# HJakeCunningham/ASVGP

Hardware: AMD Instinct MI355X
Metric: Mpoints/s per ELBO+grad step, N=10M 1D Matern-3/2 M=2048 (higher is better)
Workload: dtype f64

## Files before the change

asvgp_amd/csrc/bcr_mfma.hpp:

```cpp
#pragma once
#include "bcr.hpp"
#include "prior_plan.hpp"

namespace asvgp {

constexpr int BM_THREADS = 1024;
constexpr int BM_B = 4;
constexpr int BM_GAT = 0, BM_GBT = 16, BM_DINV = 32, BM_SD = 48, BM_CAT = 64, BM_CBT = 80, BM_W = 96, BM_DG = 100, BM_REC = 104;

__host__ __device__ inline size_t bcr_mfma_ws_doubles(long nb) { return (size_t)nb * BM_REC + 64; }
__host__ __device__ inline size_t bcr_mfma_lds_doubles(long nb) {
  return (size_t)((nb + 1) / 2 + 1) * 32 + (size_t)nb * 4 + 96 + (size_t)(BM_THREADS / 64) * 4 * 40 + (size_t)(nb / 8 + 2) * 52;
}

__device__ __forceinline__ double bm_mfma(double a, double b, double c) { return __builtin_amdgcn_mfma_f64_4x4x4f64(a, b, c, 0, 0, 0); }

__device__ __forceinline__ double bm_chol_linv(const double (&d)[10], int hi, int lo, double& dprod, int& badj) {
  double l00, i0, l10, l20, l30, l11, i1, l21, l31, l22, i2, l32, l33, i3;
  Num<double>::sqrt_inv(d[0], l00, i0);
  badj = !(d[0] > 0.0) ? 1 : 0;
  l10 = d[1] * i0; l20 = d[3] * i0; l30 = d[6] * i0;
  double s = fma(-l10, l10, d[2]);
  badj = (!(s > 0.0) && !badj) ? 2 : badj;
  Num<double>::sqrt_inv(s, l11, i1);
  l21 = fma(-l20, l10, d[4]) * i1;
  l31 = fma(-l30, l10, d[7]) * i1;
  s = fma(-l21, l21, fma(-l20, l20, d[5]));
  badj = (!(s > 0.0) && !badj) ? 3 : badj;
  Num<double>::sqrt_inv(s, l22, i2);
  l32 = fma(-l31, l21, fma(-l30, l20, d[8])) * i2;
  s = fma(-l32, l32, fma(-l31, l31, fma(-l30, l30, d[9])));
  badj = (!(s > 0.0) && !badj) ? 4 : badj;
  Num<double>::sqrt_inv(s, l33, i3);
  dprod = (l00 * l11) * (l22 * l33);
  const double z0 = (lo == 0) ? i0 : 0.0;
  const double z1 = fma(-l10, z0, (lo == 1) ? 1.0 : 0.0) * i1;
  const double z2 = fma(-l21, z1, fma(-l20, z0, (lo == 2) ? 1.0 : 0.0)) * i2;
  const double z3 = fma(-l32, z2, fma(-l31, z1, fma(-l30, z0, (lo == 3) ? 1.0 : 0.0))) * i3;
  return hi == 0 ? z0 : (hi == 1 ? z1 : (hi == 2 ? z2 : z3));
}

template <typename Src> __device__ __forceinline__ auto bm_src_load(const Src& A, int dd, long col, long M, int) -> decltype(A.load_dc(dd, col, M)) {
  return A.load_dc(dd, col, M);
}
template <typename Src> __device__ __forceinline__ double bm_src_load(const Src& A, int dd, long col, long M, long) {
  return A.load((long)dd * M + col, true);
}
struct BmLog {
  double m; int e;
  __device__ __forceinline__ void mul(double p) {
    m *= p;
    const int hi = __double2hiint(m);
    e += ((hi >> 20) & 0x7ff) - 1023;
    m = __hiloint2double((hi & 0x800fffff) | 0x3ff00000, __double2loint(m));
  }
};

__device__ __forceinline__ unsigned long long bm_wave_xor(unsigned long long x) {
#pragma unroll
  for (int off = 32; off > 0; off >>= 1) x ^= (unsigned long long)__shfl_xor((long long)x, off, 64);
  return x;
}
__device__ __forceinline__ void bm_msg_send(double* box, int n, double v, unsigned long long tag, int lane) {
  unsigned long long* b = reinterpret_cast<unsigned long long*>(box);
  const unsigned long long w = lane < n ? (unsigned long long)__double_as_longlong(v) : 0ull;
  const unsigned long long x = bm_wave_xor(w) ^ tag;
  if (lane < n) __hip_atomic_store(b + lane, w, __ATOMIC_RELAXED, __HIP_MEMORY_SCOPE_AGENT);
  if (lane == n) __hip_atomic_store(b + n, x, __ATOMIC_RELAXED, __HIP_MEMORY_SCOPE_AGENT);
}
__device__ __forceinline__ bool bm_msg_recv(const double* box, int n, double& v, unsigned long long tag, int lane, long spin_limit) {
  const unsigned long long* b = reinterpret_cast<const unsigned long long*>(box);
  for (long spins = 0; spins <= spin_limit; ++spins) {
    const unsigned long long w = lane <= n ? __hip_atomic_load(b + lane, __ATOMIC_RELAXED, __HIP_MEMORY_SCOPE_AGENT) : 0ull;
    const unsigned long long x = bm_wave_xor(lane < n ? w : 0ull) ^ tag;
    const unsigned long long chk = (unsigned long long)__shfl((long long)w, n, 64);
    if (x == chk) { v = __longlong_as_double((long long)w); return true; }
    __builtin_amdgcn_s_sleep(1);
  }
  return false;
}

struct BmSplit {
  int half = -1;
  double* xchg = nullptr;
  long spin_limit = 0;
  int* gave_up = nullptr;
  unsigned long long tag = 0;
};
constexpr int BM_XCHG = 96;

template <typename Src>
__device__ __attribute__((always_inline)) void bcr_mfma_solve(Src A, const double* rhs, int M, double* ws, double* lds, double* Sband, double* x,
                                                              double* logdet, int* info, int rhs_stride = 1, double* stamps = nullptr,
                                                              BmSplit sp = BmSplit{}) {
  constexpr int B = BM_B;
  const int tid = threadIdx.x;
  const int lane = tid & 63, wv = __builtin_amdgcn_readfirstlane(tid >> 6);
  const int r = lane >> 4, q = (lane >> 2) & 3, c = lane & 3;
  const int e = r * 4 + c, et = c * 4 + r;
  const int hi = r > c ? r : c, lo = r > c ? c : r;
  const int nb = (M + B - 1) / B;
  const int nslot = (nb + 1) / 2;
  double* Dl = lds;
  double* El = lds + (size_t)(nslot + 1) * 16;
  double* xs = El + (size_t)(nslot + 1) * 16;
  double* red = xs + (size_t)nb * B;
  double* slab = red + 96 + (size_t)(wv * 4 + q) * 40;
  double* Fl = red + 96 + (size_t)(BM_THREADS / 64) * 4 * 40;
  double* Sl = lds;
  int levels = 0;
  while ((1 << levels) < nb) ++levels;
  const bool split = sp.half >= 0;
  const int top = levels - 1, ht = 1 << (top > 0 ? top : 0);
  double s_other = 0.0;
  int bad_other = 0x7fffffff;
  auto level_share = [&](int l, int ne, int& m0, int& ne_h) {
    m0 = 0; ne_h = ne;
    if (!split) return;
    if (l < top) {
      const int mL = ht >> (l + 1);
      if (sp.half == 0) ne_h = ne < mL ? ne : mL;
      else { m0 = mL; ne_h = ne > mL ? ne - mL : 0; }
    } else {
      ne_h = sp.half == 0 ? ne : 0;
    }
  };
  int bad = 0;
  BmLog ld{1.0, 0};
  unsigned long long t_prev = stamps ? __builtin_amdgcn_s_memtime() : 0ull;
  int nst = 0;
  auto stamp = [&]() {
    if (stamps && tid == 0) { const unsigned long long t = __builtin_amdgcn_s_memtime(); stamps[nst++] = (double)(t - t_prev); t_prev = t; }
  };
  auto rec = [&](int node) -> double* { return ws + (size_t)node * BM_REC; };
  auto bandD = [&](int n, int rr, int cc) -> double {
    const int col = n * B + cc, row = n * B + rr;
    const bool pad = row >= M;
    const double v = bm_src_load(A, rr - cc, pad ? 0 : col, (long)M, 0);
    return pad ? ((rr == cc) ? 1.0 : 0.0) : v;
  };
  auto bandE = [&](int n, int rr, int cc) -> double {
    if (rr > cc) return 0.0;
    const int col = n * B + cc, row = (n + 1) * B + rr;
    const bool pad = row >= M;
    const double v = bm_src_load(A, B + rr - cc, pad ? 0 : col, (long)M, 0);
    return pad ? 0.0 : v;
  };
  if ((nb & 1) && tid < 16 && !(split && sp.half == 0)) {
    const int rr = tid >> 2, cc = tid & 3;
    Dl[(size_t)((nb - 1) >> 1) * 16 + tid] = bandD(nb - 1, rr > cc ? rr : cc, rr > cc ? cc : rr);
  }
  if (split && sp.half == 0 && tid < 16) Dl[(size_t)(ht >> 1) * 16 + tid] = 0.0;
  for (int row = tid; row < nb * B; row += BM_THREADS) {
    const bool sep_left = split && sp.half == 0 && row >= ht * B && row < (ht + 1) * B;
    xs[row] = (row < M && !sep_left) ? rhs[(long)row * rhs_stride] : 0.0;
  }
  __syncthreads();
  stamp();

  constexpr int RMAXR = 4;
  for (int l = 0; l < levels; ++l) {
    const int h = 1 << l;
    const int ne = (nb > h) ? (nb - h + 2 * h - 1) / (2 * h) : 0;
    int m0, ne_h;
    level_share(l, ne, m0, ne_h);
    if (split && l == top) {
      if (sp.half == 1) {
        if (wv == 0) {
          const double v = lane < 16 ? Dl[(size_t)(ht >> 1) * 16 + lane] : (lane < 20 ? xs[ht * B + lane - 16] : 0.0);
          bm_msg_send(sp.xchg, 20, v, sp.tag | 1ull, lane);
        }
        const double mine = (r == 0 && c == 0) ? (log(ld.m) + (double)ld.e * 0.6931471805599453094) : 0.0;
        const double tot = wave_sum_dpp(mine);
        int bm = bad ? bad : 0x7fffffff;
#pragma unroll
        for (int off = 32; off > 0; off >>= 1) { const int o = __shfl_xor(bm, off, 64); bm = o < bm ? o : bm; }
        int* sbad = reinterpret_cast<int*>(red + 32);
        if (lane == 0) { red[wv] = tot; sbad[wv] = bm; }
        __syncthreads();
        if (wv == 0) {
          double sv = 0.0;
          int bmin = 0x7fffffff;
          for (int w2 = 0; w2 < BM_THREADS / 64; ++w2) { sv += red[w2]; bmin = sbad[w2] < bmin ? sbad[w2] : bmin; }
          bm_msg_send(sp.xchg + 24, 2, lane == 0 ? sv : (double)bmin, sp.tag | 2ull, lane);
        }
      } else {
        if (wv == 0) {
          double v = 0.0;
          if (!bm_msg_recv(sp.xchg, 20, v, sp.tag | 1ull, lane, sp.spin_limit)) { if (lane == 0) *sp.gave_up = 1; }
          else {
            if (lane < 16) Dl[(size_t)(ht >> 1) * 16 + lane] += v;
            else if (lane < 20) xs[ht * B + lane - 16] += v;
          }
        }
        __syncthreads();
        if (*sp.gave_up) return;
      }
      stamp();
    }
    double updb[RMAXR], ybu[RMAXR];
    int qv = q, ev = e;
    asm volatile("" : "+v"(qv), "+v"(ev));
    double sl[2][3];
    auto slab_loads = [&](int rd0) __attribute__((always_inline)) {
#pragma unroll
      for (int u = 0; u < 2; ++u) {
#pragma unroll
        for (int t3 = 0; t3 < 3; ++t3) {
          sl[u][t3] = 0.0;
          int m = (rd0 + u) * 64 + wv * 4 + qv;
          m = m0 + (m < ne_h ? m : ne_h - 1);
          const int kk = ev + 16 * t3, dd = kk >> 3, col = m * 2 * B + (kk & 7);
          const bool in = kk < 40 && col + dd < M;
          const double v = bm_src_load(A, in ? dd : 0, in ? col : 0, (long)M, 0);
          sl[u][t3] = in ? v : ((dd == 0) ? 1.0 : 0.0);
        }
      }
    };
#pragma unroll
    for (int rd = 0; rd < RMAXR; ++rd) {
      __builtin_amdgcn_sched_barrier(0);
      if (l == 0 && (rd & 1) == 0) slab_loads(rd);
      updb[rd] = 0.0; ybu[rd] = 0.0;
      if (rd * 64 + wv * 4 >= ne_h) continue;
      const int ml = rd * 64 + wv * 4 + q;
      const bool act = ml < ne_h;
      const int i = h + (m0 + (act ? ml : ne_h - 1)) * 2 * h, a = i - h, b = i + h;
      const bool hasb = b < nb;
      const int bsafe = hasb ? b : a;
      double d[10];
      double ea, eb, da;
      if (l == 0) {
#pragma unroll
        for (int t3 = 0; t3 < 3; ++t3) if (e + 16 * t3 < 40) slab[e + 16 * t3] = sl[rd & 1][t3];
        int kk = 0;
#pragma unroll
        for (int rr = 0; rr < 4; ++rr)
#pragma unroll
          for (int cc = 0; cc <= rr; ++cc) d[kk++] = slab[(rr - cc) * 8 + 4 + cc];
        ea = slab[(4 + lo - hi) * 8 + hi];
        ea = (r <= c) ? ea : 0.0;
        eb = slab[(4 + lo - hi) * 8 + 4 + hi];
        eb = (hasb && c <= r) ? eb : 0.0;
        da = slab[(hi - lo) * 8 + lo];
      } else {
        const double* Di = Dl + (size_t)(i >> 1) * 16;
        int kk = 0;
#pragma unroll
        for (int rr = 0; rr < 4; ++rr)
#pragma unroll
          for (int cc = 0; cc <= rr; ++cc) d[kk++] = Di[rr * 4 + cc];
        ea = El[(size_t)(a >> 1) * 16 + e];
        eb = El[(size_t)(i >> 1) * 16 + et];
        eb = hasb ? eb : 0.0;
        da = Dl[(size_t)(a >> 1) * 16 + e];
      }
      double yv = xs[i * B + r], ya = xs[a * B + r];
      yv = (c == 0) ? yv : 0.0;
      ya = (c == 0) ? ya : 0.0;
      (void)bsafe;
      double dprod;
      int badj;
      const double t = bm_chol_linv(d, hi, lo, dprod, badj);
      if (act && badj && !bad) bad = i * B + badj;
      const double linv = (r >= c) ? t : 0.0;
      const double linvT = (c >= r) ? t : 0.0;
      if (act) ld.mul(dprod);
      const double ua = bm_mfma(linvT, ea, 0.0);
      const double ub = bm_mfma(linvT, eb, 0.0);
      const double zz = bm_mfma(linvT, yv, 0.0);
      const double nua = -ua, nub = -ub;
      const double da_new = bm_mfma(nua, ua, da);
      const double e_new = bm_mfma(nub, ua, 0.0);
      const double ya_new = bm_mfma(nua, zz, ya);
      updb[rd] = bm_mfma(ub, ub, 0.0);
      ybu[rd] = bm_mfma(ub, zz, 0.0);
      updb[rd] = act ? updb[rd] : 0.0;
      ybu[rd] = act ? ybu[rd] : 0.0;
      const double gat = bm_mfma(ua, linv, 0.0);
      const double gbt = bm_mfma(ub, linv, 0.0);
      const double dinv = bm_mfma(linv, linv, 0.0);
      const double w = bm_mfma(linv, zz, 0.0);
      if (act) {
        if (l >= 3) {
          double* R = Fl + (size_t)(i >> 3) * 52;
          R[e] = gat; R[16 + e] = gbt; R[32 + e] = dinv;
          if (c == 0) R[48 + r] = w;
        } else {
          double* R = rec(i);
          R[BM_GAT + e] = gat; R[BM_GBT + e] = gbt; R[BM_DINV + e] = dinv;
          if (c == 0) R[BM_W + r] = w;
        }
        Dl[(size_t)(a >> 1) * 16 + e] = da_new;
        El[(size_t)(a >> 1) * 16 + e] = e_new;
        if (c == 0) xs[a * B + r] = ya_new;
      }
    }
    bcr_lds_barrier();
#pragma unroll
    for (int rd = 0; rd < RMAXR; ++rd) {
      if (rd * 64 + wv * 4 >= ne_h) continue;
      const int ml = rd * 64 + wv * 4 + q;
      const int i = h + (m0 + ml) * 2 * h, b = i + h;
      if (ml < ne_h && b < nb) {
        Dl[(size_t)(b >> 1) * 16 + e] -= updb[rd];
        if (c == 0) xs[b * B + r] -= ybu[rd];
      }
    }
    bcr_lds_barrier();
    stamp();
  }
  if (wv == 0 && !(split && sp.half == 1)) {
    const bool act = q == 0;
    double d[10];
    int kk = 0;
#pragma unroll
    for (int rr = 0; rr < 4; ++rr)
#pragma unroll
      for (int cc = 0; cc <= rr; ++cc) { const double v = Dl[rr * 4 + cc]; d[kk++] = act ? v : ((rr == cc) ? 1.0 : 0.0); }
    const double yv = (act && c == 0) ? xs[r] : 0.0;
    double dprod;
    int badj;
    const double t = bm_chol_linv(d, hi, lo, dprod, badj);
    if (act && badj && !bad) bad = badj;
    const double linv = (r >= c) ? t : 0.0, linvT = (c >= r) ? t : 0.0;
    if (act) ld.mul(dprod);
    const double s00 = bm_mfma(linv, linv, 0.0);
    const double zz = bm_mfma(linvT, yv, 0.0);
    const double x0 = bm_mfma(linv, zz, 0.0);
    if (act) {
      rec(0)[BM_SD + e] = s00;
      Sl[e] = s00;
      if (r >= c && r < M) Sband[(long)(r - c) * M + c] = s00;
      if (c == 0) xs[r] = x0;
    }
  }
  __syncthreads();
  stamp();
  unsigned long long lw = 0ull;
  for (int l = levels - 1; l >= 0; --l) {
    const int h = 1 << l;
    const int ne = (nb > h) ? (nb - h + 2 * h - 1) / (2 * h) : 0;
    int m0, ne_h;
    level_share(l, ne, m0, ne_h);
    if (split && sp.half == 0 && wv == BM_THREADS / 64 - 1) {
      if (l == top - 1 && lane <= 2)
        lw = __hip_atomic_load(reinterpret_cast<const unsigned long long*>(sp.xchg + 24) + lane, __ATOMIC_RELAXED, __HIP_MEMORY_SCOPE_AGENT);
      if (l == 2) {
        const unsigned long long x = bm_wave_xor(lane < 2 ? lw : 0ull) ^ (sp.tag | 2ull);
        const unsigned long long chk = (unsigned long long)__shfl((long long)lw, 2, 64);
        double v = __longlong_as_double((long long)lw);
        bool ok = x == chk;
        if (!ok) ok = bm_msg_recv(sp.xchg + 24, 2, v, sp.tag | 2ull, lane, sp.spin_limit);
        if (!ok) { if (lane == 0) *sp.gave_up = 1; }
        else if (lane < 2) red[48 + lane] = v;
      }
    }
#pragma unroll
    for (int rd = 0; rd < RMAXR; ++rd) {
      __builtin_amdgcn_sched_barrier(0);
      if (rd * 64 + wv * 4 >= ne_h) continue;
      const int ml = rd * 64 + wv * 4 + q;
      const bool act = ml < ne_h;
      const int i = h + (m0 + (act ? ml : ne_h - 1)) * 2 * h, a = i - h, b = i + h;
      const bool hasb = b < nb;
      const int bs = hasb ? b : a;
      const bool e_is_a = ((a / (2 * h)) & 1) != 0;
      double gat, gbt, dinv, w, saa, sbb, sba, sab;
      if (l >= 3) {
        const double* R = Fl + (size_t)(i >> 3) * 52;
        gat = R[e]; gbt = R[16 + e]; dinv = R[32 + e]; w = R[48 + r];
      } else {
        const double* R = rec(i);
        gat = R[BM_GAT + e]; gbt = R[BM_GBT + e]; dinv = R[BM_DINV + e]; w = R[BM_W + r];
      }
      if (l >= 1) {
        const double* Ra = Sl + (size_t)(a >> 2) * 48;
        const double* Rb = Sl + (size_t)(bs >> 2) * 48;
        saa = Ra[e];
        sbb = Rb[e];
        sba = e_is_a ? Ra[32 + e] : Rb[16 + et];
        sab = e_is_a ? Ra[32 + et] : Rb[16 + e];
      } else {
        const double* Ra = rec(a);
        const double* Rb = rec(bs);
        saa = Ra[BM_SD + e];
        sbb = Rb[BM_SD + e];
        sba = e_is_a ? Ra[BM_CBT + e] : Rb[BM_CAT + et];
        sab = e_is_a ? Ra[BM_CBT + et] : Rb[BM_CAT + e];
      }
      sbb = hasb ? sbb : 0.0; sba = hasb ? sba : 0.0; sab = hasb ? sab : 0.0;
      double xa = xs[a * B + r], xb = xs[bs * B + r];
      xa = (c == 0) ? xa : 0.0;
      xb = (hasb && c == 0) ? xb : 0.0;
      w = (c == 0) ? w : 0.0;
      double ncat = bm_mfma(saa, gat, 0.0);
      ncat = bm_mfma(sba, gbt, ncat);
      double ncbt = bm_mfma(sab, gat, 0.0);
      ncbt = bm_mfma(sbb, gbt, ncbt);
      double sii = bm_mfma(ncat, gat, dinv);
      sii = bm_mfma(ncbt, gbt, sii);
      double gx = bm_mfma(gat, xa, 0.0);
      gx = bm_mfma(gbt, xb, gx);
      if (act) {
        if (c == 0) xs[i * B + r] = w - gx;
        if (l >= 2) {
          double* Rw = Sl + (size_t)(i >> 2) * 48;
          Rw[e] = sii; Rw[16 + e] = -ncat; Rw[32 + e] = -ncbt;
        }
        if (l > 0) {
          double* Rw = rec(i);
          Rw[BM_SD + e] = sii; Rw[BM_CAT + e] = -ncat; Rw[BM_CBT + e] = -ncbt;
        }
        if (r >= c && i * B + r < M) Sband[(long)(r - c) * M + i * B + c] = sii;
        if (l == 0) {
          if (c <= r && i * B + c < M) Sband[(long)(B + c - r) * M + a * B + r] = -ncat;
          if (hasb && r <= c && b * B + r < M) Sband[(long)(B + r - c) * M + i * B + c] = -ncbt;
        }
      }
    }
    if (l == 1) __syncthreads(); else bcr_lds_barrier();
    if (split && l == top) {
      double* Rs = Sl + (size_t)(ht >> 2) * 48;
      if (sp.half == 0) {
        if (wv == 0) bm_msg_send(sp.xchg + 32, 52, lane < 48 ? Rs[lane < 48 ? lane : 0] : (lane < 52 ? xs[ht * B + lane - 48] : 0.0), sp.tag | 3ull, lane);
      } else {
        if (wv == 0) {
          double v = 0.0;
          if (!bm_msg_recv(sp.xchg + 32, 52, v, sp.tag | 3ull, lane, sp.spin_limit)) { if (lane == 0) *sp.gave_up = 1; }
          else if (lane < 48) {
            Rs[lane] = v;
            rec(ht)[BM_SD + lane] = v;
            if (lane < 16) {
              const int rr = lane >> 2, cc = lane & 3;
              if (rr >= cc && ht * B + rr < M) Sband[(long)(rr - cc) * M + ht * B + cc] = v;
            }
          } else if (lane < 52) {
            xs[ht * B + lane - 48] = v;
          }
        }
        __syncthreads();
        if (*sp.gave_up) return;
      }
    }
    stamp();
  }
  if (!(split && sp.half == 0))
    for (int col = M - B + tid; col < M; col += BM_THREADS)
      if (col >= 0)
#pragma unroll
        for (int dd = 1; dd <= B; ++dd)
          if (col + dd >= M) Sband[(long)dd * M + col] = 0.0;
  {
    const int row0 = (split && sp.half == 1) ? (ht + 1) * B : 0, row1 = (split && sp.half == 0) ? (ht + 1) * B : M;
    for (int row = row0 + tid; row < row1 && row < M; row += BM_THREADS) x[(long)row * rhs_stride] = xs[row];
  }
  if (!(split && sp.half == 1)) {
    const double mine = (r == 0 && c == 0) ? (log(ld.m) + (double)ld.e * 0.6931471805599453094) : 0.0;
    const double tot = wave_sum_dpp(mine);
    int bm = bad ? bad : 0x7fffffff;
#pragma unroll
    for (int off = 32; off > 0; off >>= 1) { const int o = __shfl_xor(bm, off, 64); bm = o < bm ? o : bm; }
    int* sbad = reinterpret_cast<int*>(red + 32);
    if (lane == 0) { red[wv] = tot; sbad[wv] = bm; }
    __syncthreads();
    if (split && tid == 0) { s_other = red[48]; bad_other = (int)red[49]; }
    if (tid == 0) {
      double s = 0.0;
      int bmin = 0x7fffffff;
      for (int w2 = 0; w2 < BM_THREADS / 64; ++w2) { s += red[w2]; bmin = sbad[w2] < bmin ? sbad[w2] : bmin; }
      s += s_other;
      bmin = bad_other < bmin ? bad_other : bmin;
      __hip_atomic_store(logdet + 0, 2.0 * s, __ATOMIC_RELAXED, __HIP_MEMORY_SCOPE_AGENT);
      __hip_atomic_store(logdet + 1, 0.0, __ATOMIC_RELAXED, __HIP_MEMORY_SCOPE_AGENT);
      __hip_atomic_store(info, (bmin == 0x7fffffff) ? 0 : bmin, __ATOMIC_RELAXED, __HIP_MEMORY_SCOPE_AGENT);
    }
  }
  stamp();
}


__host__ __device__ inline size_t bcr_mfma_pre_ws_doubles(long nb) { return (size_t)nb * 96 + 64; }
__host__ __device__ inline size_t bcr_mfma_pre_lds_doubles(long nb, int n_rec) {
  return PRIOR_TAB_HEADER + (size_t)2 * n_rec * prior_rec_fields(BM_B) + (size_t)(nb / 4 + 2) * 96 + (size_t)(nb + 1) / 2 + 64;
}

struct BmDual { double v, d; };
__device__ __forceinline__ BmDual bm_dmfma(BmDual x, BmDual y, BmDual c) {
  BmDual r;
  r.v = bm_mfma(x.v, y.v, c.v);
  r.d = bm_mfma(x.d, y.v, c.d);
  r.d = bm_mfma(x.v, y.d, r.d);
  return r;
}

__device__ __attribute__((always_inline)) void bcr_mfma_backward_pre(const double* __restrict__ tab, int n_rec, const int* __restrict__ node_rec, int M,
                                                                      double* ws, double* lds, double* Sv, double* Sd, double* logdet, int* info,
                                                                      unsigned long long* done_flag, unsigned long long seq,
                                                                      const unsigned long long* ready_flag = nullptr, long spin_limit = 0, int* gave_up = nullptr) {
  constexpr int B = BM_B, W = prior_rec_fields(B);
  const int tid = threadIdx.x;
  if (ready_flag) {
    if (tid == 0) {
      long spins = 0;
      while (__hip_atomic_load(ready_flag, __ATOMIC_RELAXED, __HIP_MEMORY_SCOPE_SYSTEM) < seq) {
        __builtin_amdgcn_s_sleep(8);
        if (++spins > spin_limit) { *gave_up = 1; break; }
      }
    }
    __syncthreads();
    if (*gave_up) return;
    __builtin_amdgcn_fence(__ATOMIC_ACQUIRE, "");
  }
  const int lane = tid & 63, wv = __builtin_amdgcn_readfirstlane(tid >> 6);
  const int r = lane >> 4, q = (lane >> 2) & 3, c = lane & 3;
  const int e = r * 4 + c, et = c * 4 + r;
  const int nb = (M + B - 1) / B;
  const int n_tab = PRIOR_TAB_HEADER + 2 * n_rec * W;
  double* tl = lds;
  double* Sl = lds + n_tab;
  int* nrl = reinterpret_cast<int*>(Sl + (size_t)(nb / 4 + 2) * 96);
  {
    const double2* src = reinterpret_cast<const double2*>(tab);
    double2* dst = reinterpret_cast<double2*>(tl);
    for (int i2 = tid; i2 < n_tab / 2; i2 += BM_THREADS) dst[i2] = src[i2];
    for (int i2 = tid; i2 < nb; i2 += BM_THREADS) nrl[i2] = node_rec[i2];
  }
  __syncthreads();
  if (done_flag && tid == 0) __hip_atomic_store(done_flag, seq, __ATOMIC_RELAXED, __HIP_MEMORY_SCOPE_SYSTEM);
  const double* tv = tl + PRIOR_TAB_HEADER;
  const double* td = tv + (size_t)n_rec * W;
  int levels = 0;
  while ((1 << levels) < nb) ++levels;
  if (tid < 16) {
    const int r0 = nrl[0];
    const double xv = tv[(size_t)r0 * W + prior_f_UA(B) + tid], xd = td[(size_t)r0 * W + prior_f_UA(B) + tid];
    Sl[tid] = xv; Sl[48 + tid] = xd;
    ws[tid] = xv; ws[48 + tid] = xd;
    const int rr = tid >> 2, cc = tid & 3;
    if (rr >= cc && rr < M) { Sv[(long)(rr - cc) * M + cc] = xv; Sd[(long)(rr - cc) * M + cc] = xd; }
  }
  __syncthreads();
  constexpr int RMAXR = 4;
  for (int l = levels - 1; l >= 0; --l) {
    const int h = 1 << l;
    const int ne = (nb > h) ? (nb - h + 2 * h - 1) / (2 * h) : 0;
#pragma unroll
    for (int rd = 0; rd < RMAXR; ++rd) {
      __builtin_amdgcn_sched_barrier(0);
      if (rd * 64 + wv * 4 >= ne) continue;
      const int m = rd * 64 + wv * 4 + q;
      const bool act = m < ne;
      const int i = h + (act ? m : ne - 1) * 2 * h, a = i - h, b = i + h;
      const bool hasb = b < nb;
      const int bs = hasb ? b : a;
      const bool e_is_a = ((a / (2 * h)) & 1) != 0;
      const int ri = nrl[i];
      const double* fv = tv + (size_t)ri * W;
      const double* fd = td + (size_t)ri * W;
      const BmDual gat{fv[prior_f_GAT(B) + e], fd[prior_f_GAT(B) + e]};
      const BmDual gbt{fv[prior_f_GBT(B) + e], fd[prior_f_GBT(B) + e]};
      const BmDual dinv{fv[prior_f_DINV(B) + e], fd[prior_f_DINV(B) + e]};
      BmDual saa, sbb, sba, sab;
      if (l >= 1) {
        const double* Ra = Sl + (size_t)(a >> 2) * 96;
        const double* Rb = Sl + (size_t)(bs >> 2) * 96;
        saa = BmDual{Ra[e], Ra[48 + e]};
        sbb = BmDual{Rb[e], Rb[48 + e]};
        sba = e_is_a ? BmDual{Ra[32 + e], Ra[80 + e]} : BmDual{Rb[16 + et], Rb[64 + et]};
        sab = e_is_a ? BmDual{Ra[32 + et], Ra[80 + et]} : BmDual{Rb[16 + e], Rb[64 + e]};
      } else {
        const double* Ga = ws + (size_t)a * 96;
        const double* Gb = ws + (size_t)bs * 96;
        saa = BmDual{Ga[e], Ga[48 + e]};
        sbb = BmDual{Gb[e], Gb[48 + e]};
        sba = e_is_a ? BmDual{Ga[32 + e], Ga[80 + e]} : BmDual{Gb[16 + et], Gb[64 + et]};
        sab = e_is_a ? BmDual{Ga[32 + et], Ga[80 + et]} : BmDual{Gb[16 + e], Gb[64 + e]};
      }
      if (!hasb) { sbb = BmDual{0.0, 0.0}; sba = sbb; sab = sbb; }
      const BmDual zero{0.0, 0.0};
      BmDual ncat = bm_dmfma(saa, gat, zero);
      ncat = bm_dmfma(sba, gbt, ncat);
      BmDual ncbt = bm_dmfma(sab, gat, zero);
      ncbt = bm_dmfma(sbb, gbt, ncbt);
      BmDual sii = bm_dmfma(ncat, gat, dinv);
// ... 35 lines not shown
```

asvgp_amd/csrc/elbo.hip:

```cpp
#include <stdlib.h>
#include <time.h>
#include <string.h>

#include "bcr_pre.hpp"
#include "bcr_mfma.hpp"
#include "handle.hpp"

namespace asvgp {


struct Ws {
  double *Kuu, *dK, *P, *LK, *dLK, *LP, *SK, *dSK, *SP, *c, *alpha, *logdets, *fin, *bcrK, *bcrP;
};
static size_t bcr_ws_chain(int planes, int k, bool big) {
  long ns = 1024;
  while ((long)planes * 2 * k * k * ns * 8 + 2 * ns * k * 8 + 1024 > 150 * 1024) ns >>= 1;
  if (big) ns *= 2;
  return (size_t)planes * (7 * k * k + k) * 2 * ns + (big ? (size_t)planes * k * k * ns : 0);
}
static size_t bcr_ws_K(int k, long M) {
  size_t a = bcr_ws_chain(2, k, false), b = bcr_ws_chain(2, k, true), c = bcr_pre_ws_doubles(k, (M + k - 1) / k);
  a = a > b ? a : b;
  return (a > c ? a : c) + 64;
}
// ... 262 lines not shown
    const double v = th.v, s = th.s, N = th.N, Nw = th.Nw, Dd = (double)D;
    tot[AKA] *= alpha_scale * alpha_scale; tot[ADKA] *= alpha_scale * alpha_scale; tot[AAA] *= alpha_scale * alpha_scale;
    tot[BA] *= alpha_scale;
    if (logdets) {
      tot[LOGK] = logdets[0];
      tot[LOGP] = logdets[2];
      tot[CC] = tot[BA] / s;
    }
    const double two_pi = 6.283185307179586476925286766559;
    double elbo = -0.5 * N * Dd * log(two_pi * s);
    elbo -= 0.5 * Dd * tot[LOGP];
    elbo += 0.5 * Dd * tot[LOGK];
    elbo -= 0.5 * yy / s;
    elbo += 0.5 * tot[CC];
    elbo -= 0.5 * Nw * v / s;
    elbo += 0.5 * tot[TRKA] / s;
    if (th.cw != 0.0) elbo += th.cw;
    double d_l = 0.5 * (Dd * tot[SKDK] - Dd * tot[SPDK] - tot[ADKA] + tot[DTRKA] / s);
    double d_v = 0.5 * (-Dd * tot[SKK] / v + Dd * tot[SPK] / v + tot[AKA] / v + tot[TRKA] / (v * s)) - 0.5 * Nw / s;
    double s2 = s * s;
    double d_s = -0.5 * N * Dd / s + 0.5 * Dd * tot[SPA] / s2 + 0.5 * yy / s2 + 0.5 * tot[AAA] / s2 - tot[BA] / s2 +
                 0.5 * Nw * v / s2 - 0.5 * tot[TRKA] / s2;
    out[0] = elbo; out[1] = d_v; out[2] = d_l; out[3] = d_s;
    out[4] = tot[LOGK]; out[5] = tot[LOGP]; out[6] = tot[TRKA]; out[7] = tot[CC];
  }
#undef is_last
}

constexpr int FIN_LDS_DOUBLES = 16 * 14 + 2;

template <int KT>
__global__ __launch_bounds__(256) void elbo_finalize_kernel(
    const double* __restrict__ stats, const double* __restrict__ Kuu, const double* __restrict__ dK,
    const double* __restrict__ LK, const double* __restrict__ LP, const double* __restrict__ SK,
    const double* __restrict__ dSK, const double* __restrict__ SP, const double* __restrict__ c,
    const double* __restrict__ alpha, const double* __restrict__ logdets, long M, int k_rt, long D, ElboScalars th,
    double alpha_scale, double* __restrict__ gacc, unsigned* __restrict__ ticket, double* __restrict__ out) {
  __shared__ double part[FIN_LDS_DOUBLES];
  (void)k_rt;
  elbo_finalize_body<KT>((int)blockIdx.x, (int)gridDim.x, part, stats, Kuu, dK, LK, LP, SK, dSK, SP, c, alpha, logdets, M, D, th, alpha_scale,
                         gacc, ticket, nullptr, out);
}

struct FusedFin {
  const double* stats; ElboScalars th; double alpha_scale; double* gacc; unsigned* ticket; unsigned* arrived; unsigned* assembled; double* out;
  long D; int n_helpers; int finalize; int debug_no_assembly; int debug_stamps;
  double* mirror; unsigned long long mirror_seq;
  int split; double* xchg;
};
constexpr int FIN_GACC_PR = 21;
__device__ __forceinline__ void assemble_band_slice(const double* __restrict__ S, const double* __restrict__ coef, const double* __restrict__ dcoef, int n_terms,
                                                    long E, long e, double* __restrict__ Kuu, double* __restrict__ dK) {
#pragma clang fp contract(off)
  double sv[ASVGP_MAX_KUU_TERMS];
#pragma unroll
  for (int t = 0; t < ASVGP_MAX_KUU_TERMS; ++t) sv[t] = (t < n_terms) ? S[(long)t * E + e] : 0.0;
  double acc = coef[0] * sv[0], dacc = dcoef[0] * sv[0];
#pragma unroll
  for (int t = 1; t < ASVGP_MAX_KUU_TERMS; ++t)
    if (t < n_terms) { acc = acc + coef[t] * sv[t]; dacc = dacc + dcoef[t] * sv[t]; }
  Kuu[e] = acc;
  if (dK) dK[e] = dacc;
}
template <int K, bool BIG>
__global__ __launch_bounds__(BCR_THREADS) void elbo_chains_kernel(const double* S_static, KuuCoefs2 cf, double* Kuu, double* dK, const double* A, const double* b, int M,
                                                                  double* wsP, double* SP, double* x, double* logdets, int* info,
                                                                  double s, const double* tab, int n_rec, const int* node_rec,
                                                                  double* wsK, double* SK, double* dSK,
                                                                  unsigned long long* done_flag, unsigned long long seq, int D, int lds_doubles, FusedFin fin) {
  extern __shared__ double lds[];
  const long E = (long)(K + 1) * M;
  __shared__ int gave_up;
  if (threadIdx.x == 0) gave_up = 0;
  __syncthreads();
  if (blockIdx.x == 0) {
    if (threadIdx.x == 0) {
      long spins = 0;
      while (__hip_atomic_load(fin.assembled, __ATOMIC_RELAXED, __HIP_MEMORY_SCOPE_AGENT) < (unsigned)fin.n_helpers) {
        __builtin_amdgcn_s_sleep(2);
        if (++spins > (1L << 25)) { gave_up = 1; break; }
      }
      if (!gave_up) __hip_atomic_store(fin.assembled, 0u, __ATOMIC_RELAXED, __HIP_MEMORY_SCOPE_AGENT);
    }
    __syncthreads();
    if (gave_up) { if (threadIdx.x == 0) atomicExch(info + 1, -1); return; }
    __builtin_amdgcn_fence(__ATOMIC_ACQUIRE, "agent");
    bcr_solve<double, K, 1, BandSumP, BIG>(BandSumP{A, Kuu, 1.0 / s}, b, M, wsP, lds, BandOut<double>{SP, nullptr}, x, logdets + 2, info + 1, nullptr, D);
    more_columns<K, BIG>(b, x, D, M, wsP, lds, lds_doubles);
  } else if (blockIdx.x == 1) {
    bcr_backward_pre<K>(tab, n_rec, node_rec, M, wsK, lds, BandOut<Dual>{SK, dSK}, logdets, info, done_flag, seq);
  } else {
    for (long e = (long)(blockIdx.x - 2) * blockDim.x + threadIdx.x; e < E; e += (long)fin.n_helpers * blockDim.x)
      assemble_band_slice(S_static, cf.c, cf.dc, cf.n, E, e, Kuu, dK);
    __syncthreads();
    if (threadIdx.x == 0) {
      __threadfence();
      __hip_atomic_fetch_add(fin.assembled, 1u, __ATOMIC_RELEASE, __HIP_MEMORY_SCOPE_AGENT);
    }
  }
  if (!fin.finalize) return;
  if (blockIdx.x < 2) {
    __syncthreads();
    if (threadIdx.x == 0) {
      __threadfence();
      __hip_atomic_fetch_add(fin.arrived, 1u, __ATOMIC_RELEASE, __HIP_MEMORY_SCOPE_AGENT);
    }
    return;
  }
  if (threadIdx.x == 0) {
    long spins = 0;
    while (__hip_atomic_load(fin.arrived, __ATOMIC_RELAXED, __HIP_MEMORY_SCOPE_AGENT) < 2u) {
      __builtin_amdgcn_s_sleep(8);
      if (++spins > (1L << 25)) { gave_up = 1; break; }
    }
  }
  __syncthreads();
  if (gave_up) { if (threadIdx.x == 0) atomicExch(info + 1, -1); return; }
  __builtin_amdgcn_fence(__ATOMIC_ACQUIRE, "agent");
  elbo_finalize_body<K>((int)blockIdx.x - 2, fin.n_helpers, lds, fin.stats, Kuu, dK, nullptr, nullptr, SK, dSK, SP, nullptr, x, logdets, (long)M, fin.D,
                        fin.th, fin.alpha_scale, fin.gacc, fin.ticket, fin.arrived, fin.out);
}

template <int K>
__global__ __launch_bounds__(BM_THREADS) void elbo_chains_mfma_kernel(KuuInterior ki, const double* S_static, KuuCoefs2 cf, double* Kuu, double* dK, const double* A, const double* b, int M,
                                                                      double* wsP, double* SP, double* x, double* logdets, int* info,
                                                                      double s, const double* tab, int n_rec, const int* node_rec,
                                                                      double* wsK, double* SK, double* dSK,
                                                                      unsigned long long* done_flag, unsigned long long seq,
                                                                      const unsigned long long* ready_flag, long spin_limit, FusedFin fin, const ThetaBox* box) {
  extern __shared__ double lds[];
  static_assert(K == BM_B, "matrix-core chains: bandwidth 4");
  const long E = (long)(K + 1) * M;
  const unsigned long long t_start = fin.debug_stamps ? __builtin_amdgcn_s_memrealtime() : 0ull;
  auto rstamp = [&](int slot) {
    if (fin.debug_stamps && threadIdx.x == 0 && blockIdx.x <= 2)
      logdets[(slot < 4 ? 8 + 4 * (int)blockIdx.x : 24) + slot] = (slot == 0) ? (double)(t_start & 0xffffffffull) : (double)((__builtin_amdgcn_s_memrealtime() - t_start) & 0xffffffffull);
  };
  rstamp(0);
  __shared__ int gave_up, kuu_ok;
  __shared__ double kuu_pref[4];
  if (threadIdx.x == 0) { gave_up = 0; kuu_ok = 0; }
  __syncthreads();
  double s_v = s, asc_v = fin.alpha_scale;
  ElboScalars th_v = fin.th;
  if (box) {
    if (threadIdx.x == 0) {
      long spins = 0;
      for (;;) {
        const unsigned long long got = __hip_atomic_load(&box->seq, __ATOMIC_RELAXED, __HIP_MEMORY_SCOPE_SYSTEM);
        if (got == seq) break;
        if (got == ~0ull || ++spins > spin_limit) { gave_up = 1; break; }
        __builtin_amdgcn_s_sleep(2);
      }
    }
    __syncthreads();
    if (gave_up) { if (threadIdx.x == 0) atomicExch(info + 1, -1); return; }
    s_v = box->s; asc_v = box->alpha_scale;
    th_v.v = box->v; th_v.l = box->l; th_v.s = box->s; th_v.N = box->N; th_v.Nw = box->Nw; th_v.cw = box->cw;
  }
  const double* stats = fin.stats;
  enum { LOGK, LOGP, TRKA, DTRKA, SKDK, SPDK, SKK, SPK, SPA, CC, AKA, ADKA, AAA, BA, NACC };
  double acc[NACC];
#pragma unroll
  for (int i = 0; i < NACC; ++i) acc[i] = 0.0;
  const bool isP = blockIdx.x == 0 || (fin.split && blockIdx.x == 2);
  const bool isPR = fin.split && blockIdx.x == 2;
  __shared__ double kdl[16];
  __shared__ double bnd[2 * PRIOR_BND_DIAGS * PRIOR_BND], dkb[2 * 5 * KI_DKB];
  {
    if (isP) rstamp(1);
    if (threadIdx.x == 0) {
      if (box) {
#pragma unroll
        for (int i = 0; i < 5; ++i) { kdl[i] = box->k[i]; kdl[8 + i] = box->dk[i]; }
      } else {
        kdl[0] = ki.k[0]; kdl[1] = ki.k[1]; kdl[2] = ki.k[2]; kdl[3] = ki.k[3]; kdl[4] = ki.k[4];
        kdl[8] = ki.dk[0]; kdl[9] = ki.dk[1]; kdl[10] = ki.dk[2]; kdl[11] = ki.dk[3]; kdl[12] = ki.dk[4];
      }
    }
    {
      const double* bnd_g = box ? box->bnd : reinterpret_cast<const double*>((const char*)__builtin_amdgcn_kernarg_segment_ptr() + offsetof(KuuInterior, bnd));
      const double* dkb_g = box ? box->dkb : reinterpret_cast<const double*>((const char*)__builtin_amdgcn_kernarg_segment_ptr() + offsetof(KuuInterior, dkb));
      if (threadIdx.x < 2 * PRIOR_BND_DIAGS * PRIOR_BND) bnd[threadIdx.x] = bnd_g[threadIdx.x];
      else if (threadIdx.x < 2 * PRIOR_BND_DIAGS * PRIOR_BND + 2 * 5 * KI_DKB) dkb[threadIdx.x - 2 * PRIOR_BND_DIAGS * PRIOR_BND] = dkb_g[threadIdx.x - 2 * PRIOR_BND_DIAGS * PRIOR_BND];
    }
    __syncthreads();
  }
  if (isP) {
    BmSplit bsp;
    if (fin.split) { bsp.half = isPR ? 1 : 0; bsp.xchg = fin.xchg; bsp.spin_limit = spin_limit; bsp.gave_up = &gave_up; bsp.tag = seq << 8; }
    bcr_mfma_solve<BandSumToep>(BandSumToep{A, 1.0 / s_v, (lds_cdouble_ptr)kdl, (lds_cdouble_ptr)bnd, ki.lo, ki.hi}, b, M, wsP, lds, SP, x, logdets + 2, info + 1, 1,
                                fin.debug_stamps ? (isPR ? fin.xchg + 128 : logdets + 32) : (double*)nullptr, bsp);
    rstamp(3);
    __syncthreads();
    if (gave_up) { if (threadIdx.x == 0) atomicExch(info + 1, -1); return; }
    rstamp(4);
    if (fin.finalize) {
      const double* xs_l = lds + (size_t)2 * ((((M + K - 1) / K) + 1) / 2 + 1) * 16;
      static_assert(BM_THREADS == 1024, "two columns per thread");
      int nbl = (M + K - 1) / K, lv = 0;
      while ((1 << lv) < nbl) ++lv;
      const long jsep = (long)(1 << (lv > 0 ? lv - 1 : 0)) * K;
      const long j0 = isPR ? jsep : 0, j1 = (fin.split && !isPR) ? jsep : (long)M;
      unsigned long long kw = 0ull;
      const bool kuu_reader = !isPR && (threadIdx.x >> 6) == 1;
      if (kuu_reader && (threadIdx.x & 63) <= 4)
        kw = __hip_atomic_load(reinterpret_cast<const unsigned long long*>(fin.gacc + 8) + (threadIdx.x & 63), __ATOMIC_RELAXED, __HIP_MEMORY_SCOPE_AGENT);
      double sp[2][K + 1], av[2][K + 1], bj[2];
#pragma unroll
      for (int cI = 0; cI < 2; ++cI) {
        const long j = j0 + threadIdx.x + cI * BM_THREADS, jc = j < j1 ? j : j1 - 1;
#pragma unroll
        for (int r = 0; r <= K; ++r) { sp[cI][r] = SP[(long)r * M + jc]; av[cI][r] = stats[(long)r * M + jc]; }
        bj[cI] = stats[(long)(K + 1) * M + jc];
      }
#pragma unroll
      for (int cI = 0; cI < 2; ++cI) {
        const long j = j0 + threadIdx.x + cI * BM_THREADS;
        if (j >= j1) continue;
        const bool left = j < ki.lo, right = j >= ki.hi;
        const double xj = xs_l[j];
#pragma unroll
        for (int r = 0; r <= K; ++r) {
          const long o = (long)r * M + j;
          const double w2 = (r == 0) ? 1.0 : 2.0;
          double kv = kdl[r], dkv = kdl[8 + r];
          if (left || right) {
            kv = bnd[left ? (long)r * PRIOR_BND + j : (long)(PRIOR_BND_DIAGS + r) * PRIOR_BND + (j - ki.hi)];
            if (ki.dk_tab) {
              dkv = dkb[left ? (long)r * KI_DKB + j : (long)(5 + r) * KI_DKB + (j - ki.hi)];
            } else {
              dkv = 0.0;
              for (int t = 0; t < cf.n; ++t) dkv = fma(box ? box->dc[t] : cf.dc[t], S_static[(long)t * E + o], dkv);
            }
          }
          const double xx = (j + r < M) ? w2 * xj * xs_l[j + r] : 0.0;
          acc[SPDK] = fma(w2 * sp[cI][r], dkv, acc[SPDK]);
          acc[SPK] = fma(w2 * sp[cI][r], kv, acc[SPK]);
          acc[SPA] = fma(w2 * sp[cI][r], av[cI][r], acc[SPA]);
          acc[AKA] = fma(kv, xx, acc[AKA]);
          acc[ADKA] = fma(dkv, xx, acc[ADKA]);
          acc[AAA] = fma(av[cI][r], xx, acc[AAA]);
        }
        acc[BA] = fma(bj[cI], xj, acc[BA]);
      }
      if (kuu_reader) {
        const int ln = threadIdx.x & 63;
        const unsigned long long x = bm_wave_xor(ln < 4 ? kw : 0ull) ^ ((seq << 8) | 4ull);
        const unsigned long long chk = (unsigned long long)__shfl((long long)kw, 4, 64);
        if (x == chk) { if (ln < 4) kuu_pref[ln] = __longlong_as_double((long long)kw); if (ln == 0) kuu_ok = 1; }
      }
    }
  } else {
    if (fin.debug_no_assembly) {
      if (threadIdx.x == 0) { for (long sp_ = 0; sp_ < spin_limit; ++sp_) __builtin_amdgcn_s_sleep(8); atomicExch(info + 1, -1); }
      return;
    }
    bcr_mfma_backward_pre(tab, n_rec, node_rec, M, wsK, lds, SK, dSK, logdets, info, done_flag, seq, ready_flag,
                          spin_limit < (1L << 20) ? spin_limit : (1L << 20), &gave_up);
    if (gave_up) { if (threadIdx.x == 0) atomicExch(info + 1, -1); return; }
    rstamp(1);
    if (fin.finalize) {
      __syncthreads();
      double sk[2][K + 1], dsk[2][K + 1], av[2][K + 1];
#pragma unroll
      for (int cI = 0; cI < 2; ++cI) {
        const long j = (long)threadIdx.x + cI * BM_THREADS, jc = j < M ? j : M - 1;
#pragma unroll
        for (int r = 0; r <= K; ++r) { sk[cI][r] = SK[(long)r * M + jc]; dsk[cI][r] = dSK[(long)r * M + jc]; av[cI][r] = stats[(long)r * M + jc]; }
      }
#pragma unroll
      for (int cI = 0; cI < 2; ++cI) {
        const long j = (long)threadIdx.x + cI * BM_THREADS;
        if (j >= M) continue;
        const bool left = j < ki.lo, right = j >= ki.hi;
#pragma unroll
        for (int r = 0; r <= K; ++r) {
          const long o = (long)r * M + j;
          const double w2 = (r == 0) ? 1.0 : 2.0;
          double kv = kdl[r], dkv = kdl[8 + r];
          if (left || right) {
            kv = bnd[left ? (long)r * PRIOR_BND + j : (long)(PRIOR_BND_DIAGS + r) * PRIOR_BND + (j - ki.hi)];
            if (ki.dk_tab) {
              dkv = dkb[left ? (long)r * KI_DKB + j : (long)(5 + r) * KI_DKB + (j - ki.hi)];
            } else {
              dkv = 0.0;
              for (int t = 0; t < cf.n; ++t) dkv = fma(box ? box->dc[t] : cf.dc[t], S_static[(long)t * E + o], dkv);
            }
          }
          acc[TRKA] = fma(w2 * sk[cI][r], av[cI][r], acc[TRKA]);
          acc[DTRKA] = fma(w2 * dsk[cI][r], av[cI][r], acc[DTRKA]);
          acc[SKDK] = fma(w2 * sk[cI][r], dkv, acc[SKDK]);
          acc[SKK] = fma(w2 * sk[cI][r], kv, acc[SKK]);
        }
      }
    }
  }
  if (!fin.finalize) { rstamp(2); return; }
  if (isP) rstamp(5);
  double* part0 = lds;
  const int lane = threadIdx.x & 63;
  double mine[8];
  mine[0] = isP ? acc[SPDK] : acc[TRKA];
  mine[1] = isP ? acc[SPK] : acc[DTRKA];
  mine[2] = isP ? acc[SPA] : acc[SKDK];
  mine[3] = isP ? acc[AKA] : acc[SKK];
// ... 816 lines not shown
```

Measured before the change: 134,500.

## Keep level-1 and root BCR selected-inverse blocks in LDS instead of global workspace

The level-0 back-substitution of the MFMA block cyclic reduction used to read the selected-inverse blocks (diag, cat, cbt) of levels 0 and 1 from the global workspace records. Those blocks now go to an LDS region (S1) that reuses the tail of the scratch area, sized to the larger of the two uses. This drops the global writes and reads and lets the level-1 full __syncthreads become a cheaper LDS barrier. An acquire fence is also added after the mailbox spin in the finalize kernel, a correctness fix that costs a little. The cost is a larger LDS footprint and aliasing with the slab and Fl scratch, which depends on those no longer being live at that point.

```diff
diff --git a/asvgp_amd/csrc/bcr_mfma.hpp b/asvgp_amd/csrc/bcr_mfma.hpp
--- a/asvgp_amd/csrc/bcr_mfma.hpp
+++ b/asvgp_amd/csrc/bcr_mfma.hpp
@@ -6,11 +6,12 @@
 
 constexpr int BM_THREADS = 1024;
 constexpr int BM_B = 4;
-constexpr int BM_GAT = 0, BM_GBT = 16, BM_DINV = 32, BM_SD = 48, BM_CAT = 64, BM_CBT = 80, BM_W = 96, BM_DG = 100, BM_REC = 104;
+constexpr int BM_GAT = 0, BM_GBT = 16, BM_DINV = 32, BM_W = 96, BM_REC = 104;
 
 __host__ __device__ inline size_t bcr_mfma_ws_doubles(long nb) { return (size_t)nb * BM_REC + 64; }
 __host__ __device__ inline size_t bcr_mfma_lds_doubles(long nb) {
-  return (size_t)((nb + 1) / 2 + 1) * 32 + (size_t)nb * 4 + 96 + (size_t)(BM_THREADS / 64) * 4 * 40 + (size_t)(nb / 8 + 2) * 52;
+  const size_t tail = (size_t)(BM_THREADS / 64) * 4 * 40 + (size_t)(nb / 8 + 2) * 52, lvl1 = (size_t)(nb / 4 + 2) * 48;
+  return (size_t)((nb + 1) / 2 + 1) * 32 + (size_t)nb * 4 + 96 + (tail > lvl1 ? tail : lvl1);
 }
 
 __device__ __forceinline__ double bm_mfma(double a, double b, double c) { return __builtin_amdgcn_mfma_f64_4x4x4f64(a, b, c, 0, 0, 0); }
@@ -108,6 +109,7 @@
   double* slab = red + 96 + (size_t)(wv * 4 + q) * 40;
   double* Fl = red + 96 + (size_t)(BM_THREADS / 64) * 4 * 40;
   double* Sl = lds;
+  double* S1 = red + 96;
   int levels = 0;
   while ((1 << levels) < nb) ++levels;
   const bool split = sp.half >= 0;
@@ -329,7 +331,6 @@
     const double zz = bm_mfma(linvT, yv, 0.0);
     const double x0 = bm_mfma(linv, zz, 0.0);
     if (act) {
-      rec(0)[BM_SD + e] = s00;
       Sl[e] = s00;
       if (r >= c && r < M) Sband[(long)(r - c) * M + c] = s00;
       if (c == 0) xs[r] = x0;
@@ -338,6 +339,10 @@
   __syncthreads();
   stamp();
   unsigned long long lw = 0ull;
+  int m0_1 = 0, ne_1 = 0;
+  if (levels > 1) level_share(1, (nb > 2) ? (nb + 1) / 4 : 0, m0_1, ne_1);
+  (void)ne_1;
+  double* S1rel = S1 - (size_t)m0_1 * 48;
   for (int l = levels - 1; l >= 0; --l) {
     const int h = 1 << l;
     const int ne = (nb > h) ? (nb - h + 2 * h - 1) / (2 * h) : 0;
@@ -374,20 +379,13 @@
         const double* R = rec(i);
         gat = R[BM_GAT + e]; gbt = R[BM_GBT + e]; dinv = R[BM_DINV + e]; w = R[BM_W + r];
       }
-      if (l >= 1) {
-        const double* Ra = Sl + (size_t)(a >> 2) * 48;
-        const double* Rb = Sl + (size_t)(bs >> 2) * 48;
+      {
+        const double* Ra = ((a & 2) ? S1rel : Sl) + (size_t)(a >> 2) * 48;
+        const double* Rb = ((bs & 2) ? S1rel : Sl) + (size_t)(bs >> 2) * 48;
         saa = Ra[e];
         sbb = Rb[e];
         sba = e_is_a ? Ra[32 + e] : Rb[16 + et];
         sab = e_is_a ? Ra[32 + et] : Rb[16 + e];
-      } else {
-        const double* Ra = rec(a);
-        const double* Rb = rec(bs);
-        saa = Ra[BM_SD + e];
-        sbb = Rb[BM_SD + e];
-        sba = e_is_a ? Ra[BM_CBT + e] : Rb[BM_CAT + et];
-        sab = e_is_a ? Ra[BM_CBT + et] : Rb[BM_CAT + e];
       }
       sbb = hasb ? sbb : 0.0; sba = hasb ? sba : 0.0; sab = hasb ? sab : 0.0;
       double xa = xs[a * B + r], xb = xs[bs * B + r];
@@ -404,13 +402,9 @@
       gx = bm_mfma(gbt, xb, gx);
       if (act) {
         if (c == 0) xs[i * B + r] = w - gx;
-        if (l >= 2) {
-          double* Rw = Sl + (size_t)(i >> 2) * 48;
+        if (l >= 1) {
+          double* Rw = (l >= 2 ? Sl : S1rel) + (size_t)(i >> 2) * 48;
           Rw[e] = sii; Rw[16 + e] = -ncat; Rw[32 + e] = -ncbt;
-        }
-        if (l > 0) {
-          double* Rw = rec(i);
-          Rw[BM_SD + e] = sii; Rw[BM_CAT + e] = -ncat; Rw[BM_CBT + e] = -ncbt;
         }
         if (r >= c && i * B + r < M) Sband[(long)(r - c) * M + i * B + c] = sii;
         if (l == 0) {
@@ -419,7 +413,7 @@
         }
       }
     }
-    if (l == 1) __syncthreads(); else bcr_lds_barrier();
+    bcr_lds_barrier();
     if (split && l == top) {
       double* Rs = Sl + (size_t)(ht >> 2) * 48;
       if (sp.half == 0) {
@@ -430,7 +424,6 @@
           if (!bm_msg_recv(sp.xchg + 32, 52, v, sp.tag | 3ull, lane, sp.spin_limit)) { if (lane == 0) *sp.gave_up = 1; }
           else if (lane < 48) {
             Rs[lane] = v;
-            rec(ht)[BM_SD + lane] = v;
             if (lane < 16) {
               const int rr = lane >> 2, cc = lane & 3;
               if (rr >= cc && ht * B + rr < M) Sband[(long)(rr - cc) * M + ht * B + cc] = v;
diff --git a/asvgp_amd/csrc/elbo.hip b/asvgp_amd/csrc/elbo.hip
--- a/asvgp_amd/csrc/elbo.hip
+++ b/asvgp_amd/csrc/elbo.hip
@@ -438,6 +438,7 @@
         if (got == ~0ull || ++spins > spin_limit) { gave_up = 1; break; }
         __builtin_amdgcn_s_sleep(2);
       }
+      __builtin_amdgcn_fence(__ATOMIC_ACQUIRE, "");
     }
     __syncthreads();
     if (gave_up) { if (threadIdx.x == 0) atomicExch(info + 1, -1); return; }
```

New measurement: 129,500. 0.963x the previous value.
